# Blaok/soda

Hardware: AMD Instinct MI355X
Metric: stencil cells*iters/s, jacobi2d 8192x8192 iterate=100 (higher is better)
Workload: dtype f32; 1 GPU; jacobi2d float 8192x8192 iterate=100; kernel_family=march2d, decomposition=none, overlap=False, transport=none

## Files before the change

soda_amd/codegen/hip/lower.py:

```python
import dataclasses
import os
from typing import Dict, Optional, Sequence, Union

from soda_amd import core, util

from soda_amd.codegen.hip.module import (KernelDesc, Module, PassDesc,
                                         _check_native, runtime_text)
from soda_amd.codegen.hip.direct import DIRECT_BLOCK, add_direct_pass
from soda_amd.codegen.hip.ldswin import (add_ldswin_pass,
                                         ldswin_candidate, ldswin_pays,
                                         ldswin_supported)
from soda_amd.codegen.hip.march import (LANE_SHIFTS, MAX_FUSE_3D,
                                        MAX_FUSE_PRESERVE, MAX_SHIFT_TEMPS,
                                        MAX_UNROLL, REG_BUDGET, MarchConfig,
                                        add_march_pass, default_vec,
                                        march_supported)
from soda_amd.codegen.hip.tile3d import (add_tile3d_pass,
                                         tile3d_supported)


MAX_TENSORS = 16
DEFAULT_FUSE = (13, 12, 8, 4)
SLIDING_SUMS = os.environ.get('SODA_HIP_SLIDE', '1') != '0'

# ... 5 lines not shown
class LowerOptions:

  strategy: str = 'auto'
  fuse: Sequence[int] = (4,)
  vec: Optional[int] = None
  chunk_rows: Optional[int] = None
  prefetch: Optional[int] = None
  waves_x: int = 1
  waves_y: int = 1
  nt_store: Optional[bool] = None
  nt_load: Optional[bool] = None
  xcd_swizzle: bool = True
  edge_loads: bool = True
  tile_rows: Optional[int] = None
  lane_shift: Optional[str] = None
  min_waves: int = 0
  occupancy: int = 0
  pipe: Optional[int] = None
  pipe_rows: int = 2
  reg_budget: Optional[int] = None
  stamps: bool = False
  peel: Union[None, int, Dict[int, int]] = None
  align_lanes: Optional[int] = None
  xshare: Optional[bool] = None
  row_cells: Optional[int] = None
  xshare_block: Optional[int] = None
  windows: Optional[bool] = None
  inline: Optional[bool] = None
  tile3d_w: Optional[int] = None
  tile3d_h: Optional[int] = None
  tile3d_waves: Optional[int] = None
  banks: Optional[Dict[str, int]] = None
  bank_lead: Optional[Dict[str, int]] = None
  batch: bool = False

  def __post_init__(self):
    self.fuse = tuple(self.fuse)
    if self.inline is None:
      self.inline = os.environ.get('SODA_HIP_INLINE', '1') != '0'
    if self.windows is None:
      self.windows = os.environ.get('SODA_HIP_WINDOWS', '1') != '0'
    if self.xshare is None and os.environ.get('SODA_HIP_XSHARE'):
      self.xshare = os.environ['SODA_HIP_XSHARE'] == '1'
    if self.xshare_block is None and os.environ.get('SODA_HIP_XSHARE_BLOCK'):
      self.xshare_block = int(os.environ['SODA_HIP_XSHARE_BLOCK'])
    if self.align_lanes is None and os.environ.get('SODA_HIP_ALIGN_LANES'):
      self.align_lanes = int(os.environ['SODA_HIP_ALIGN_LANES'])

  def resolved(self, dim: int, iterated: bool = True) -> 'LowerOptions':
    out = dataclasses.replace(self)
    if out.prefetch is None and dim == 3:
      out.prefetch = 1
    if out.nt_load is None:
      out.nt_load = dim != 3 and iterated
    if out.nt_store is None:
      out.nt_store = not iterated
    if out.tile_rows is None:
      out.tile_rows = 4
    return out


NARROW_STRIP_OPS = (48, 128)


def prefers_narrow_strips(stencil: core.Stencil) -> bool:
  if os.environ.get('SODA_HIP_NARROW', '1') == '0':
    return False
  if stencil.dim != 2 or stencil.iterate != 1:
    return False
  if any(str(t) != 'float' for t in stencil.symbol_table.values()):
    return False
  from soda_amd import ir as _ir
  work = sum(_ir.op_count(s.stmt.expr) +
             sum(_ir.op_count(l.expr) for l in s.stmt.let)
             for s in stencil.ordered_stages)
  return NARROW_STRIP_OPS[0] <= work < NARROW_STRIP_OPS[1]


# ... 83 lines not shown
      skip = ((0, None),) + (((stencil.dim - 1, '+'),) if SLIDING_SUMS else ())
    derived = windows.decompose(stencil, skip=skip)
    if len(derived.symbol_table) + len(derived.param_stmts) <= MAX_TENSORS \
        and same_boxes(derived):
      stencil = derived
  from soda_amd.codegen.hip import exact
  stencil = exact.specialize(stencil)
  mod = Module(stencil, opts.banks, opts.batch)
  use_march = opts.strategy in ('auto', 'march', 'tile3d') and \
      march_supported(stencil) is None
  if opts.strategy == 'march' and not use_march:
    raise util.SemanticError('march: %s' % march_supported(stencil))
  if use_march:
    vec0 = opts.vec or default_vec(stencil)
    iterable = (len(stencil.input_names) == len(stencil.output_names) and
                stencil.input_types == stencil.output_types)
    cap = stencil.iterate
    if stencil.dim == 3 and opts.strategy != 'march':
      cap = min(cap, MAX_FUSE_3D)
    if stencil.preserve_border and opts.strategy != 'march':
      cap = min(cap, MAX_FUSE_PRESERVE)
    depths = sorted({min(t, cap) for t in opts.fuse if iterable} - {0, 1},
                    reverse=True)
    if opts.strategy == 'tile3d':
      depths = []

    def peel_for(t: int) -> int:
      if opts.peel is None:
        return -1
      if isinstance(opts.peel, dict):
        return int(opts.peel.get(t, -1))
      return int(opts.peel)

    def pipe_for(t: int) -> int:
      want = default_pipe(t) if opts.pipe is None else opts.pipe
      ok = (want > 1 and t > 1 and t % want == 0 and
            opts.waves_x * opts.waves_y == 1)
      return want if ok else 1

    out_bytes = min(t.size_in_bytes for t in stencil.output_types)

    def shift_for(t: int, xshare: int = 0) -> str:
      if opts.lane_shift is not None:
        return opts.lane_shift
      if xshare or pipe_for(t) > 1 or opts.waves_x * opts.waves_y != 1:
        return 'dpp'
      return default_lane_shift(t, stencil.dim)

    def config(t: int, vec: int, pf: Optional[int],
               rows: Optional[int] = None, xshare: int = 0,
               xshare_block: int = 0) -> MarchConfig:
      shift = shift_for(t, xshare or xshare_block)
      if pf is None:
        pf = default_prefetch(t, shift)
      if opts.align_lanes is not None:
        align = opts.align_lanes
      else:
        align = max(1, 64 // (vec * out_bytes)) if opts.nt_store else 1
      cfg = MarchConfig(
          fused_iters=t, vec=vec, chunk_rows=opts.chunk_rows or 64,
          prefetch=pf, waves_x=opts.waves_x, waves_y=opts.waves_y,
          nt_store=opts.nt_store, nt_load=opts.nt_load,
          xcd_swizzle=opts.xcd_swizzle, edge_loads=opts.edge_loads,
          tile_rows=rows or opts.tile_rows, lane_shift=shift,
          min_waves=opts.min_waves, occupancy=opts.occupancy,
          pipe=pipe_for(t), pipe_rows=opts.pipe_rows, stamps=opts.stamps,
          peel=peel_for(t), align_lanes=align, xshare=xshare,
          xshare_block=xshare_block,
          xwindow=bool(opts.windows),
          slide=bool(opts.windows) and SLIDING_SUMS,
          banks=opts.banks, bank_lead=opts.bank_lead)
      cfg.chunk_fixed = opts.chunk_rows is not None
      return cfg

    budget = opts.reg_budget or REG_BUDGET
    first = default_prefetch(1) if stencil.dim == 2 and work < 128 else \
        (2 if stencil.dim == 2 else 1)
    pfs = [opts.prefetch] if opts.prefetch else [first, 2, 1]
    pfs = sorted(set(pfs), reverse=True)
    rows_list = [opts.tile_rows]
    vecs = []
    v = vec0
    while v >= 1:
      vecs.append(v)
      v //= 2
    chosen = None
    last_error = None
    for v in vecs:
      for rows in rows_list:
        for pf in pfs:
          trial = Module(stencil, opts.banks, opts.batch)
          try:
            est = add_march_pass(trial, config(1, v, pf, rows)).traffic_model[
                'est_window_regs']
          except util.SemanticError as e:
            last_error = e
            continue
          if chosen is None or est < chosen[0]:
            chosen = (est, v, pf, rows)
          if est <= budget:
            break
# ... 73 lines not shown
```

soda_amd/codegen/hip/march.py:

```python
from typing import Dict, List, Optional, Tuple

from soda_amd import core, ir, util

from soda_amd.codegen.hip.module import KernelDesc, Module, PassDesc

MAX_UNROLL = 24
MAX_FUSE_PRESERVE = 8
MAX_FUSE_3D = 2
MAX_SHIFT_TEMPS = 64
REG_BUDGET = 160


class _Node:

  def __init__(self, key, ctype: str, stage: Optional[core.Stage], it: int):
    self.key = key
    self.ctype = ctype
    self.stage = stage
    self.it = it
    self.parents: Dict[str, '_Node'] = {}
    self.delay = 0
    self.first_use = None
    self.window = 1
    self.slots = 1
# ... 25 lines not shown
  @property
  def fill_delay(self) -> int:
    if self.mirror_of is not None:
      return self.delay - MIRROR_PREFETCH
    return 0 if self.stage is None else self.delay

  @property
  def var(self) -> str:
    if self.mirror_of is not None:
      return 'm%d_%s' % (self.owner, self.mirror_of.var)
    if self.stage is None:
      return 'g_%s' % self.key[1]
    return 't%d_%s' % (self.it, self.stage.name)


LDS_PER_CU = 160 * 1024
MIRROR_PREFETCH = 1


LANE_SHIFTS = {'dpp': '', 'mixh': '_mixh'}


class MarchConfig:

  def __init__(self, *, fused_iters: int = 1, vec: int = 4, chunk_rows: int = 64,
               prefetch: int = 2, waves_x: int = 1, waves_y: int = 1,
               nt_store: bool = False, nt_load: bool = True,
               xcd_swizzle: bool = True, edge_loads: bool = True,
               tile_rows: int = 6, lane_shift: str = 'dpp',
               min_waves: int = 0, occupancy: int = 0,
               pipe: int = 1, pipe_rows: int = 4, stamps: bool = False,
               peel: int = -1, align_lanes: int = 1, xshare: int = 0,
               xwindow: bool = True, slide: bool = True,
               xshare_block: int = 0,
               banks: Optional[Dict[str, int]] = None,
               bank_lead: Optional[Dict[str, int]] = None):
    self.banks = dict(banks or {})
    self.bank_lead = {n: int(v) for n, v in (bank_lead or {}).items() if v}
    self.xwindow = xwindow
    self.slide = slide
    self.xshare = int(xshare)
    self.xshare_block = int(xshare_block)
    self.align_lanes = max(1, int(align_lanes))
    self.peel = int(peel)
    self.stamps = stamps
    self.pipe_rows = pipe_rows if pipe > 1 else 1
    self.pipe = pipe
    self.occupancy = occupancy
    self.min_waves = min_waves
    self.lane_shift = lane_shift
    self.fused_iters = fused_iters
    self.vec = vec
    self.chunk_rows = chunk_rows
    self.prefetch = prefetch
    self.waves_x = waves_x
    self.waves_y = waves_y
    self.nt_store = nt_store
    self.nt_load = nt_load
    self.xcd_swizzle = xcd_swizzle
    self.edge_loads = edge_loads
    self.tile_rows = tile_rows
    self.chunk_fixed = False

  def key(self) -> str:
    return ''.join((
        'T%d_V%d_P%d_W%dx%d_R%d' % (self.fused_iters, self.vec, self.prefetch,
                                    self.waves_x, self.waves_y, self.tile_rows),
        '_nts' if self.nt_store else '', '_ntl' if self.nt_load else '',
        '_xcd' if self.xcd_swizzle else '', '_edge' if self.edge_loads else '',
        LANE_SHIFTS[self.lane_shift],
        '_mw%d' % self.min_waves if self.min_waves else '',
        '_occ%d' % self.occupancy if self.occupancy else '',
        '_buf',
        '_pipe%dx%d' % (self.pipe, self.pipe_rows) if self.pipe > 1 else '',
        '_st' if self.stamps else '',
        '_k%d' % self.peel if self.peel >= 0 else '',
        '_al%d' % self.align_lanes if self.align_lanes > 1 else '',
        '_xs%d' % self.xshare if self.xshare and not self.xshare_block
        else '',
        '_xb%d' % self.xshare_block if self.xshare_block else '',
        '_bk_' + '_'.join('%sx%d' % (n, nb) + (
            'l%d' % self.bank_lead[n] if n in self.bank_lead else '')
                         for n, nb in sorted(self.banks.items()))
        if self.banks else ''))


def default_vec(stencil: core.Stencil) -> int:
  widest = max(t.size_in_bytes for t in stencil.symbol_table.values())
  return max(1, 16 // widest)


def bank_fragment_map(vec: int, nb: int) -> List[Tuple[int, int]]:
  if nb < 1 or vec % nb:
    raise util.SemanticError(
        'banks: %d cells per lane are no whole number of groups of %d banks' %
        (vec, nb))
  return [(j % nb, j // nb) for j in range(vec)]


def edge_cell_banks(i: int, vec: int, nb: int) -> Tuple[int, int]:
  if nb < 1 or vec % nb:
    raise util.SemanticError('banks: %d cells per lane, %d banks' % (vec, nb))
  return (-1 - i) % nb, (vec + i) % nb


def march_supported(stencil: core.Stencil) -> Optional[str]:
  if stencil.dim not in (2, 3):
    return 'the marching kernels need a 2- or 3-dimensional program'
  return None


def _build_chain(st: core.Stencil, T: int, pf: int, edge: Tuple[int, int],
                 pipe: int = 1, pipe_rows: int = 1, xshare: bool = False):
# ... 128 lines not shown

  def __init__(self, mod: Module, cfg: MarchConfig):
    self.mod, self.cfg = mod, cfg
    self.st = self.mod.stencil
    why = march_supported(self.st)
    if why:
      raise util.SemanticError('march: %s' % why)
    self.dim = self.st.dim
    self.ax = self.dim - 1
    self.T, self.V, self.PF = self.cfg.fused_iters, self.cfg.vec, self.cfg.prefetch
    if self.T > 1 and len(self.st.input_names) != len(self.st.output_names):
      raise util.SemanticError('march: cannot fuse iterations of a program '
                               'whose inputs and outputs differ in number')
    self.edge = (0, 0)
    self.group = 32 if self.cfg.lane_shift == 'mixh' else 64
    if self.cfg.edge_loads and self.cfg.lane_shift == 'dpp':
      lo = hi = 0
      for stage in self.st.ordered_stages:
        for pname in stage.taps:
          if pname in self.st.input_names:
            tlo, thi = stage.tap_bounds(pname)
            lo, hi = max(lo, -tlo[0]), max(hi, thi[0])
      if max(lo, hi) <= min(self.V, 2):
        self.edge = (lo, hi)
    self.W = self.cfg.pipe
    if self.W > 1:
      if self.T % self.W or self.cfg.waves_x * self.cfg.waves_y != 1:
        raise util.SemanticError(
            'march: %d pipelined waves need a fusion depth that is a multiple '
            'of it and one strip per block' % self.W)
      self.edge = (0, 0)
    self.R = self.cfg.pipe_rows if self.W > 1 else 1
    self.banks = self.cfg.banks
    for nme, nb in self.banks.items():
      if self.mod.banks.get(nme) != nb:
        raise util.InternalError('march: banks of `%s` and the module\'s slots '
                                 'differ' % nme)
      if self.W > 1:
        raise util.SemanticError(
            'march: stage-pipelined blocks read and write dense arrays')
      bank_fragment_map(self.V, nb)
    for nme in self.cfg.bank_lead:
      if nme not in self.banks or nme not in self.st.input_names or \
          self.cfg.bank_lead[nme] % self.banks[nme] or \
          self.cfg.bank_lead[nme] < 0:
        raise util.SemanticError(
            'march: bank_lead of `%s`: a banked input, a multiple of its bank '
            'count' % nme)
    if self.R & (self.R - 1):
      raise util.SemanticError('march: rows per barrier must be a power of two')
    self.xs = self.cfg.xshare
    self.seg = bool(self.cfg.xshare_block)
    if self.seg:
      if not 2 <= self.cfg.xshare_block <= 16:
        raise util.SemanticError(
            'march: xshare_block = %d: 2 to 16 waves share a segment of a row'
            % self.cfg.xshare_block)
      self.xs = self.cfg.xshare_block
    if self.xs:
      self.edge = (0, 0)
      if self.W > 1 or self.cfg.lane_shift != 'dpp' or \
          self.cfg.waves_x * self.cfg.waves_y != 1:
        raise util.SemanticError(
            'march: x-halo sharing needs DPP shifts and one wave per strip')
      if not 1 <= self.xs <= 16:
        raise util.SemanticError('march: 1 to 16 waves can share a row')
# ... 173 lines not shown
    self.w('}')
    return self._finish()

  def _emit_header(self) -> None:
    self.w('// %s: T=%d fused iteration(s), %d cells/lane, chunks of %d along dim %d,'
      ' prefetch %d, unroll %d' % (self.kind, self.T, self.V,
                                   self.cfg.chunk_rows, self.ax, self.PF,
                                   self.U))
    self.w('// strip: %d lanes valid of 64 (halo %d+%d cells, edge loads %d+%d); '
      'pipeline depth %d' % (self.strip_lanes, self.margin_lo, self.margin_hi,
                             self.edge[0], self.edge[1],
                             self.warm))
    if self.seg:
      self.w('// segment: %d waves side by side store %d cells; x-halos shared '
             'through LDS between them, %d+%d halo lanes at the outer sides' %
             (self.xs, self.seg_cells, self.lanes_lo, self.lanes_hi))
    for nme, nb in sorted(self.banks.items()):
      self.w('// banked: %s on %d banks (a.buf[%d..%d]), cell j of a fragment = '
             'element j / %d of bank j %% %d%s' %
             (nme, nb, self.mod.slot[nme], self.mod.slot[nme] + nb - 1, nb, nb,
              ', read %d elements on' % self.cfg.bank_lead[nme]
              if nme in self.cfg.bank_lead else ''))
    if self.dim == 3:
      self.w('// tile: %d rows held in registers for %d output rows (halo %d+%d)' %
        (self.rows_in, self.tile_rows, self.rhalo_lo, self.rhalo_hi))
    for n in self.nodes:
      self.w('//   %-24s delay %2d  window %2d (slots %2d)  margin %d/%d  rows %d/%d' %
        (n.var, n.delay, n.window, n.slots, n.margin[0], n.margin[1],
         n.rmargin[0], n.rmargin[1]))
    self.w('extern "C" __global__ void __launch_bounds__(%d) %s%s(soda_hip_kargs_t a) {'
      % (self.block, '__attribute__((amdgpu_waves_per_eu(%d, %d))) ' %
         (self.cfg.min_waves, max(self.cfg.min_waves, 8))
         if self.cfg.min_waves else '', self.name))
    if self.cfg.stamps:
      self.w('  const unsigned long long soda_t0 = __builtin_amdgcn_s_memtime();')
    self.w('  const int lane = (int)(threadIdx.x & 63u);')
    self.w('  const int wave = __builtin_amdgcn_readfirstlane((int)(threadIdx.x >> 6));')
    if self.cfg.xcd_swizzle:
      self.w('  const unsigned nblk = gridDim.x;')
      self.w('  const unsigned bid = (nblk % 8u == 0u) ? (blockIdx.x % 8u) * (nblk / 8u)'
        ' + blockIdx.x / 8u : blockIdx.x;')
    else:
      self.w('  const unsigned bid = blockIdx.x;')
    self.w('  const int tile_x = (int)(bid % (unsigned)a.ntile[0]);')
    if self.dim == 2:
      self.w('  const int tile_l = (int)(bid / (unsigned)a.ntile[0]);')
      self.w('  const int tile_m = tile_l + (tile_l >= a.skip_from ? a.skip_count : 0);')
      if self.xs:
        self.w('  const int strip = wave;')
        self.w('  const int chunk = tile_m;')
      elif self.W > 1:
        self.w('  const int strip = tile_x;')
        self.w('  const int chunk = tile_m;')
      else:
        self.w('  const int strip = tile_x * %d + wave %% %d;' % (self.wx, self.wx))
        self.w('  const int chunk = tile_m * %d + wave / %d;' % (self.cfg.waves_y, self.wx))
      self.w('  const int n0 = a.extent[0], nm = a.extent[1];')
    else:
      self.w('  const int tile_y = (int)((bid / (unsigned)a.ntile[0]) % '
        '(unsigned)a.ntile[1]);')
      self.w('  const int chunk_l = (int)(bid / ((unsigned)a.ntile[0] * '
        '(unsigned)a.ntile[1]));')
      self.w('  const int chunk = chunk_l + (chunk_l >= a.skip_from ? a.skip_count : 0);')
      self.w('  const int strip = %s;' % ('wave' if self.xs else 'tile_x'))
      self.w('  const int n0 = a.extent[0], n1 = a.extent[1], nm = a.extent[2];')
      self.w('  const int y0 = tile_y * %d - %d;  // first row held' %
# ... 8 lines not shown
      self.w('  const int x0 = strip * %d + (lane - %d) * %d;' %
        (self.strip_cells, self.lanes_lo, self.V))
    else:
      self.w('  const int sub = lane & %d;' % (self.group - 1))
      self.w('  const int x0 = strip * %d + (lane >> 5) * %d + (sub - %d) * %d;'
        % (self.strip_cells, self.group_lanes * self.V, self.lanes_lo, self.V))
    self.w('  const int chunk_len = a.tile[%d] / %d;' %
      (self.ax, self.cfg.waves_y if self.dim == 2 else 1))
    self.w('  const int m_begin = chunk * chunk_len;')
    self.w('  const int m_end = min(m_begin + chunk_len, nm);')
    if self.xs:
      self.w('  if (m_begin >= nm) return;  // block-uniform')
    else:
      self.w('  if (m_begin >= nm || strip * %d >= n0) return;  // wave-uniform' %
        self.strip_cells)
    self.w('  const bool lane_ok = x0 >= 0 && x0 + %d <= n0;' % self.V)
    if self.seg:
      self.w('  const bool store_ok = lane_ok && (strip > 0 || sub >= %d) && '
             '(strip < %d || sub < %d);' %
             (self.lanes_lo, self.xs - 1, 64 - self.lanes_hi))
    else:
      self.w('  const bool store_ok = lane_ok && sub >= %d && sub < %d;' %
        (self.lanes_lo, self.group - self.lanes_hi))
    self.w('  const int64_t pitch = a.stride[%d];' % self.ax)
    self.w('  const int64_t x0c = lane_ok ? (int64_t)x0 : 0;')

  def _emit_addressing(self) -> None:
    table0 = self.st.symbol_table
    self.esz = {nme: table0[nme].size_in_bytes for nme in list(self.inputs) + list(self.outputs)}
    self.n_edge = max(self.edge)
    self.w('  const int in_end = min(nm, m_end + %d);  // last input plane needed + 1'
      % self.m_hi)
    self.w('  const int wlo = max(0, m_begin + (%d));' % self.m_lo)
    for es in sorted(set(self.esz.values())):
      self.w('  const unsigned xb%d = lane_ok ? (unsigned)x0 * %du : SODA_OOB_X;' %
        (es, es))
      self.w('  const unsigned sxb%d = store_ok ? (unsigned)x0 * %du : SODA_OOB_X;' %
        (es, es))
      self.w('  const unsigned pitch_b%d = (unsigned)pitch * %du;' % (es, es))
      if self.dim == 3:
        self.w('  const unsigned pitch_yb%d = (unsigned)pitch_y * %du;' % (es, es))
        for j in range(self.rows_in):
          self.w('  const unsigned yo%d_%d = (y0 + %d >= 0 && y0 + %d < n1) ? '
                 '(unsigned)(y0 + %d) * pitch_yb%d : SODA_OOB_X;' %
                 (es, j, j, j, j, es))
    for nme, n in self.inputs.items():
      if nme in self.banks:
        nb, lead = self.banks[nme], self.cfg.bank_lead.get(nme, 0)
        size = '(int64_t)(in_end - wlo) * pitch'
        if lead:
          self.w('  const int64_t left_%s = (int64_t)a.reserved[0] - %d - '
                 '(int64_t)wlo * pitch;  // elements of the stream from wlo on'
                 % (nme, lead))
          size = '(%s < left_%s ? %s : left_%s)' % (size, nme, size, nme)
        for b in range(nb):
          self.w('  const soda_rsrc_t r_%s_b%d = soda_make_rsrc_bank<%d>((const '
                 '%s*)a.buf[%d] + ((int64_t)wlo * pitch + %d) / %d, %s * %d);' %
                 (nme, b, nb, n.ctype, self.mod.slot[nme] + b, lead, nb, size,
                  self.esz[nme]))
        continue
      self.w('  const soda_rsrc_t r_%s = soda_make_rsrc((const %s*)a.buf[%d] + '
        '(int64_t)wlo * pitch, (int64_t)(in_end - wlo) * pitch * %d);' %
        (nme, n.ctype, self.mod.slot[nme], self.esz[nme]))
    for o, n in self.outputs.items():
      if o in self.banks:
        nb = self.banks[o]
        for b in range(nb):
          self.w('  const soda_rsrc_t w_%s_b%d = soda_make_rsrc_bank<%d>((%s*)'
                 'a.buf[%d] + ((int64_t)m_begin * pitch) / %d, (int64_t)(m_end - '
                 'm_begin) * pitch * %d);' %
                 (o, b, nb, n.ctype, self.mod.slot[o] + b, nb, self.esz[o]))
        continue
      self.w('  const soda_rsrc_t w_%s = soda_make_rsrc((%s*)a.buf[%d] + '
        '(int64_t)m_begin * pitch, (int64_t)(m_end - m_begin) * pitch * %d);' %
        (o, n.ctype, self.mod.slot[o], self.esz[o]))
    if self.xs or self.n_edge:
      self.w('  const bool edge_lane = lane == 0 || lane == 63;')
    self.xs_nodes = [n for n in self.nodes if n.xs]
    if self.xs_nodes:
      self.xs_rows = max(len(self.rows_of(n)) for n in self.xs_nodes)
      if self.xs_rows > 32:
        raise util.SemanticError('march: x-halo sharing holds a row per lane')
      self.xs_stride = self.xs * 2 * self.xs_rows
      for n in self.xs_nodes:
        self.w('  __shared__ %s soda_xs_%s[%d];' %
               (n.ctype, n.var, 2 * self.xs_stride + 1))
      self.w('  if (threadIdx.x == 0) {')
      for n in self.xs_nodes:
        self.w('    soda_xs_%s[%d] = (%s)0;' % (n.var, 2 * self.xs_stride, n.ctype))
      self.w('  }')
      self.w('  soda_pipe_barrier();')
      self.w('  const int xs_wr = (wave * 2 + (lane == 0 ? 0 : 1)) * %d;' %
             self.xs_rows)
      self.w('  const int xs_nb = lane < 32 ? wave - 1 : wave + 1;')
      self.w('  const int xs_rd = (xs_nb >= 0 && xs_nb < %d && (lane & 31) < %d) ? '
             '(xs_nb * 2 + (lane < 32 ? 1 : 0)) * %d + (lane & 31) : %d;' %
             (self.xs, self.xs_rows, self.xs_rows, 2 * self.xs_stride))
    if self.n_edge:
      for i in range(self.n_edge):
        self.w('  const int ex%d = lane == 0 ? x0 - %d : x0 + %d;' %
          (i, 1 + i, self.V + i))
        self.w('  const bool edge_ok%d = edge_lane && ex%d >= 0 && ex%d < n0;' %
          (i, i, i))
        for es in sorted({self.esz[nme] for nme in self.inputs}):
          self.w('  const unsigned exb%d_%d = edge_ok%d ? (unsigned)ex%d * %du : '
            'SODA_OOB_X;' % (i, es, i, i, es))

    if self.st.preserve_border:
      for o in self.st.output_names:
        wlo, whi = self.st.interior_bounds(o)
        for e in range(self.V):
          self.w('  const bool keepx_%s_%d = !(a.origin[0] + x0 + %d >= %d && '
                 'a.origin[0] + x0 + %d < a.gextent[0] - %d);'
                 % (o, e, e, max(0, -wlo[0]), e, max(0, whi[0])))
    self.use_mix = self.cfg.lane_shift == 'mixh'
    self.slide: Dict[int, Tuple[str, Tuple[int, ...], int]] = {}
    if self.cfg.xwindow and self.cfg.slide and self.W == 1:
      from soda_amd.optimization import windows
      table = dict(self.st.symbol_table)
      for n in self.nodes:
        if n.stage is None or n.mirror_of is not None or n.keep is not None:
          continue
        m = windows._match(n.stage.stmt, table)
        if m is None or m[0] != '+' or m[2] != self.ax:
          continue
        off = tuple(a - b for a, b in zip(m[5], n.stage.st_idx))
        self.slide[id(n)] = (m[1], off, m[4])
    declared = set()
    for stage in self.st.ordered_stages:
      for line in self.mod.param_decls(stage):
        if line not in declared:
          declared.add(line)
          self.w(line)
    for n in self.nodes:
      if n.to_lds:
        self.w('  __shared__ %s soda_ring_%s[%d][%d][%d];' % (
            n.ctype, n.var, 2 * self.R, self.rows_in, 64 * self.V))
    self.nt_l = 'true' if self.cfg.nt_load else 'false'
    self.nt_s = 'true' if self.cfg.nt_store else 'false'

  def emit_decls(self, wv: int) -> None:
      for n in self.nodes:
        if n.owner != wv:
          continue
        if id(n) in self.slide:
          for j in self.rows_of(n):
            self.w('  int xa_%s_r%d[%d];' % (n.var, j, self.V))
            self.w('  soda_zero_frag<int, %d>(xa_%s_r%d);' % (self.V, n.var, j))
        for s in range(n.slots):
          for j in self.rows_of(n):
            self.w('  %s %s_s%d_r%d[%d];' % (n.ctype, n.var, s, j, self.V))
            self.w('  soda_zero_frag<%s, %d>(%s_s%d_r%d);' % (n.ctype, self.V, n.var, s, j))
            if n.is_input and self.n_edge:
              self.w('  %s %s_s%d_r%d_e[%d];' % (n.ctype, n.var, s, j, self.n_edge))
              self.w('  soda_zero_frag<%s, %d>(%s_s%d_r%d_e);' %
                (n.ctype, self.n_edge, n.var, s, j))
          if n.xs:
            self.w('  %s hv_%s_s%d = (%s)0;' % (n.ctype, n.var, s, n.ctype))

  def emit_loads(self, k: int, t_expr: str, pin: bool = False) -> None:
      self.w('      const int t = %s;' % t_expr)
      self.w('      const bool plane_ok = t >= 0 && t < in_end;')
      if pin:
        for es in sorted({self.esz[nme] for nme in self.inputs}):
          self.w('      unsigned xb%dp = xb%d; asm volatile("" : "+v"(xb%dp));'
                 % (es, es, es))
      pinned = 'p' if pin else ''
      for es in sorted({self.esz[nme] for nme in self.inputs}):
        if self.dim == 2:
          self.w('      const unsigned ro%d = plane_ok ? (unsigned)(t - wlo) * '
            'pitch_b%d : SODA_OOB_ROW;' % (es, es))
        else:
          self.w('      const unsigned po%d = plane_ok ? (unsigned)(t - wlo) * '
            'pitch_b%d : SODA_OOB_X;' % (es, es))
          for j in sorted({j for n in self.inputs.values() for j in self.rows_of(n)}):
            self.w('      const unsigned ro%d_%d = po%d + yo%d_%d;' %
                   (es, j, es, es, j))
      for nme, n in self.inputs.items():
        s = self.slot_of(n, k, 0)
        for j in self.rows_of(n):
          es = self.esz[nme]
          ro = 'ro%d' % es if self.dim == 2 else 'ro%d_%d' % (es, j)
          reg = '%s_s%d_r%d' % (n.var, s, j)
          if nme in self.banks:
            nb = self.banks[nme]
            self.w('      soda_buf_load_frag_banked<%s, %d, %d, %s>(%s, %s + '
                   'xb%d%s, %s);' %
                   (n.ctype, self.V, nb, self.nt_l, reg, ro, es, pinned,
                    ', '.join('r_%s_b%d' % (nme, b) for b in range(nb))))
            for i in range(self.n_edge):
              left, right = edge_cell_banks(i, self.V, nb)
              self.w('      { %s e1[1], e2[1]; soda_buf_load_cell_banked<%s, %d>('
                     'e1, r_%s_b%d, lane == 0 ? %s + exb%d_%d : SODA_OOB_X); '
                     'soda_buf_load_cell_banked<%s, %d>(e2, r_%s_b%d, lane == 0 '
                     '? SODA_OOB_X : %s + exb%d_%d); %s_e[%d] = lane == 0 ? '
                     'e1[0] : e2[0]; }' %
                     (n.ctype, n.ctype, nb, nme, left, ro, i, es,
                      n.ctype, nb, nme, right, ro, i, es, reg, i))
            continue
          self.w('      soda_buf_load_frag<%s, %d, %s>(%s, r_%s, %s + xb%d%s);' %
            (n.ctype, self.V, self.nt_l, reg, nme, ro, es, pinned))
          for i in range(self.n_edge):
# ... 58 lines not shown
    self._wide: Dict[str, str] = {}
    self._stage_mark = len(self.L)
    fresh_xs: List[Tuple[_Node, int]] = []
    if self.xs and wv == 0:
      for n in self.inputs.values():
        if n.xs:
          fresh_xs.append((n, self.slot_of(n, k, self.PF)))
      for n in self.nodes:
        if not n.xs:
          continue
        slot = self.slot_of(n, k - 1, self.PF if n.is_input else 0)
        self.w('      hv_%s_s%d = soda_xs_%s[xs_rd < %d ? xs_rd + ((t - 1) & 1) * %d '
               ': xs_rd];' % (n.var, slot, n.var, 2 * self.xs_stride,
                              self.xs_stride))
    for n in self.nodes:
      if n.stage is not None and n.owner == wv:
        if step is not None and not self.stage_needed(n, step):
          continue
        first = step is not None and (step == 0 or
                                      not self.stage_needed(n, step - 1))
        self._emit_stage(n, k, slide_init='first' if first else None)
        if n.xs:
          fresh_xs.append((n, self.slot_of(n, k, 0)))
    self.shift_temps = max(self.shift_temps, len(self._shifted))
    if fresh_xs:
      self.w('      if (edge_lane) {')
      for n, slot in fresh_xs:
        for jj, j in enumerate(self.rows_of(n)):
          reg = '%s_s%d_r%d' % (n.var, slot, j)
          self.w('        soda_xs_%s[xs_wr + (t & 1) * %d + %d] = lane == 0 ? %s[0] '
                 ': %s[%d];' % (n.var, self.xs_stride, jj, reg, reg, self.V - 1))
      self.w('      }')
      self.w('      soda_pipe_barrier();')
    self.w('    }')

  def _emit_stage(self, n: _Node, k: int,
                  slide_init: Optional[str] = None) -> None:
    stage = n.stage
    pre: List[str] = []
    early: List[str] = []

    def operand(pname: str, off: Tuple[int, ...], j: int, e: int, _n=n,
                _k=k, _pre=pre, _early=early) -> str:
      p = _n.parents[pname]
      age = _n.delay - off[self.ax] - p.fill_delay
      slot = self.slot_of(p, _k, age)
      row = j + (off[1] if self.dim == 3 else 0)
      if row < p.rmargin[0] or row >= self.rows_in - p.rmargin[1]:
        raise util.InternalError('march: row %d of %s is not held' %
                                 (row, p.var))
      reg = '%s_s%d_r%d' % (p.var, slot, row)
      c = e + off[0]
      lane_off, sub = c // self.V, c % self.V
      src = '%s[%d]' % (reg, sub)
      byte = p.ctype in ('uint8_t', 'int8_t')

      def wide(text: str, tag: str) -> str:
        if not byte:
          return text
        if tag not in self._wide:
          self._wide[tag] = 'w%d_%s' % (len(self._wide), tag)
          _pre.append('      const int %s = soda_wide(%s);' %
                      (self._wide[tag], text))
        return self._wide[tag]

      if lane_off == 0:
# ... 171 lines not shown
            mid = '%s((%s)%s, %s)' % (fn, pt, c, mid)
          body.append('        const %s xm_%s = %s;' % (pt, btag, mid))
          suf = {}
          prev = None
          for i in range(lo - 1, e0 - 1, -1):
            name = 'xs_%s_%d' % (btag, i)
            expr = '(%s)%s' % (pt, cells[i]) if prev is None else \
                '%s((%s)%s, %s)' % (fn, pt, cells[i], prev)
            body.append('        const %s %s = %s;' % (pt, name, expr))
            suf[i] = prev = name
          pre = {}
          prev = None
          for i in range(hi + 1, e0 + b + taps - 1):
            name = 'xp_%s_%d' % (btag, i)
            expr = '(%s)%s' % (pt, cells[i]) if prev is None else \
                '%s(%s, (%s)%s)' % (fn, prev, pt, cells[i])
            body.append('        const %s %s = %s;' % (pt, name, expr))
            pre[i] = prev = name
          for e in range(e0, e0 + b):
            parts = ['xm_%s' % btag]
            if e < lo:
              parts.append(suf[e])
            if e + taps - 1 > hi:
              parts.append(pre[e + taps - 1])
            expr = parts[0]
            for q in parts[1:]:
              expr = '%s(%s, %s)' % (fn, expr, q)
            body.append('        %s = (%s)(%s);' % (dst[e], n.ctype, expr))
      body.append('      }')

  def _emit_store(self, n: _Node, oname: str, dst_slot: int) -> None:
    es = self.esz[oname]
    self.w('      {')
    self.w('        const int m = t - %d;' % n.delay)
    self.w('        const bool m_ok = m >= m_begin && m < m_end;')
    for j in self.store_rows(n):
      reg = '%s_s%d_r%d' % (n.var, dst_slot, j)
      if oname in self.banks:
        nb = self.banks[oname]
        off = ('(m_ok ? (unsigned)(m - m_begin) * pitch_b%d : SODA_OOB_X) + '
               'yo%d_%d + sxb%d' % (es, es, j, es)) if self.dim == 3 else (
                   '(m_ok ? (unsigned)(m - m_begin) * pitch_b%d : SODA_OOB_ROW) '
                   '+ sxb%d' % (es, es))
        self.w('        soda_buf_store_frag_banked<%s, %d, %d, %s>(%s, %s, %s);' %
               (n.ctype, self.V, nb, self.nt_s, off, reg,
                ', '.join('w_%s_b%d' % (oname, b) for b in range(nb))))
        continue
      if self.dim == 3:
        self.w('        soda_buf_store_frag<%s, %d, %s>(w_%s, (m_ok ? (unsigned)'
          '(m - m_begin) * pitch_b%d : SODA_OOB_X) + yo%d_%d + sxb%d, %s);' %
          (n.ctype, self.V, self.nt_s, oname, es, es, j, es, reg))
      else:
        self.w('        soda_buf_store_frag<%s, %d, %s>(w_%s, (m_ok ? '
          '(unsigned)(m - m_begin) * pitch_b%d : SODA_OOB_ROW) + sxb%d, '
          '%s);' % (n.ctype, self.V, self.nt_s, oname, es, es, reg))
    self.w('      }')

  def _finish(self) -> PassDesc:
    if self.shift_temps > MAX_SHIFT_TEMPS:
      raise util.SemanticError(
          'march: %d lane-shifted operands per row step (> %d); the taps reach '
          'too far along dim 0 for %d cells per lane' %
          (self.shift_temps, MAX_SHIFT_TEMPS, self.V))
    self.est_regs += self.shift_temps
    stages = [n for n in self.nodes if n.stage is not None]
    per_wave = []
# ... 7 lines not shown
        wide = 2.0 if n.ctype in ('double', 'int64_t', 'uint64_t') else 1.0
        ops += cost * wide * self.V * len(self.rows_of(n))
      per_wave.append(ops + 8.0)
    step_ops = max(per_wave)
    saved = sum(1 for i in range(self.peeled) for n in stages
                if not self.stage_needed(n, i)) / float(max(1, len(stages)))
    if self.dim == 2:
      tile = (self.strip_cells * (self.xs or self.wx),
              self.cfg.chunk_rows * self.cfg.waves_y)
    else:
      tile = (self.strip_cells * (self.xs or 1), self.tile_rows,
              self.cfg.chunk_rows)
    if self.seg:
      tile = (self.seg_cells,) + tile[1:]
    lds_pad = 0
    if self.cfg.occupancy:
      blocks_per_cu = max(1, 4 * self.cfg.occupancy // self.waves)
      lds_pad = min(65536, (LDS_PER_CU // (blocks_per_cu + 1)) // 1024 * 1024
                    + 1024)
    idx = self.mod.add_kernel(
        KernelDesc(self.name, (self.block, 1, 1), tile, lds_bytes=lds_pad,
                   note='%s %s' % (self.kind, self.cfg.key()),
                   tune=dict(axis=self.ax, waves_along=self.cfg.waves_y if self.dim == 2 else 1,
                             waves_per_block=self.waves, warm=self.warm,
                             fixed=self.cfg.chunk_fixed, occupancy=self.cfg.occupancy,
                             pipe=self.W, vec=self.V, step_ops=step_ops,
                             lane_shift=self.cfg.lane_shift,
                             warm_saved=saved,
                             lane_redundancy=self.lane_redundancy,
                             peel_trips=self.peeled // self.U,
                             unroll=self.U, tile_rows=self.tile_rows,
                             peel_trips_max=self.peel_trips_max,
                             fused=self.T,
                             window_extra=self.m_hi - self.m_lo,
                             max_elem=max(self.esz.values()),
                             max_extent0=0 if self.seg else
                             self.strip_cells * self.xs)),
        '\n'.join(self.L) + '\n')
    table = self.st.symbol_table
    bytes_in = sum(table[i].size_in_bytes for i in self.st.input_names)
    bytes_out = sum(table[o].size_in_bytes for o in self.st.output_names)
    redundancy = self.lane_redundancy * (
        (self.cfg.chunk_rows + self.warm) / float(self.cfg.chunk_rows)) * (
            self.rows_in / float(self.tile_rows))
    p = PassDesc(
        self.T, [idx], self.kind,
        dict(bytes_per_cell_min=bytes_in + bytes_out,
             read_redundancy=redundancy, strip_cells=self.strip_cells, warm_rows=self.warm,
             unroll=self.U, edge=self.edge, rows_in=self.rows_in, tile_rows=self.tile_rows,
             est_window_regs=self.est_regs))
    self.mod.passes.append(p)
    return p


def add_march_pass(mod: Module, cfg: MarchConfig) -> PassDesc:
  return _MarchKernel(mod, cfg).emit()
```

soda_amd/csrc/soda_rt.h:

```cpp

#ifdef __HIPCC_RTC__
typedef __INT8_TYPE__ int8_t;
typedef __UINT8_TYPE__ uint8_t;
typedef __INT16_TYPE__ int16_t;
typedef __UINT16_TYPE__ uint16_t;
typedef __INT32_TYPE__ int32_t;
typedef __UINT32_TYPE__ uint32_t;
typedef __INT64_TYPE__ int64_t;
typedef __UINT64_TYPE__ uint64_t;
#else
#include <hip/hip_runtime.h>
#include <stdint.h>
#endif

struct soda_hip_kargs_t {
  void* buf[16];
  int64_t stride[4];
  int32_t extent[4];
  int32_t ntile[4];
  int32_t tile[4];
  int32_t origin[4];
  int32_t gextent[4];
  int32_t skip_from;
  int32_t skip_count;
// ... 228 lines not shown
    for (int e = 0; e < V; ++e) dst[e] = t[e];
  }
}

template <class T, int V>
SODA_DEV void soda_zero_frag(T (&dst)[V]) {
#pragma unroll
  for (int e = 0; e < V; ++e) dst[e] = (T)0;
}

template <class T, int V, bool kNonTemporal = false>
SODA_DEV void soda_store_frag(T* __restrict__ p, const T (&src)[V]) {
  if constexpr (V == 1) {
    if constexpr (kNonTemporal) __builtin_nontemporal_store(src[0], p);
    else *p = src[0];
  } else {
    typedef typename soda_vec<T, V>::type vec_t;
    vec_t t;
#pragma unroll
    for (int e = 0; e < V; ++e) t[e] = src[e];
    if constexpr (kNonTemporal)
      __builtin_nontemporal_store(t, reinterpret_cast<vec_t*>(p));
    else
      *reinterpret_cast<vec_t*>(p) = t;
  }
}

typedef unsigned soda_u32x4 __attribute__((ext_vector_type(4)));
typedef unsigned soda_u32x2 __attribute__((ext_vector_type(2)));
typedef __amdgpu_buffer_rsrc_t soda_rsrc_t;
#define SODA_OOB_X 0x40000000u
#define SODA_OOB_ROW 0x80000000u
#define SODA_BUF_WINDOW_MAX 0x40000000ll

SODA_DEV soda_rsrc_t soda_make_rsrc(const void* base, int64_t bytes) {
  return __builtin_amdgcn_make_buffer_rsrc(
      const_cast<void*>(base), 0,
      (int)(bytes < 0 ? 0 : bytes > SODA_BUF_WINDOW_MAX ? SODA_BUF_WINDOW_MAX
                                                        : bytes),
      0x00020000);
}

template <class T, int V, bool kNonTemporal = false>
SODA_DEV void soda_buf_load_frag(T (&dst)[V], soda_rsrc_t r, unsigned off) {
  constexpr int kBytes = V * (int)sizeof(T);
  constexpr int kAux = kNonTemporal ? 2 : 0;
  if constexpr (kBytes % 16 == 0) {
#pragma unroll
    for (int i = 0; i < kBytes / 16; ++i) {
      const soda_u32x4 t =
          __builtin_amdgcn_raw_buffer_load_b128(r, off + 16 * i, 0, kAux);
      __builtin_memcpy((char*)dst + 16 * i, &t, 16);
    }
  } else if constexpr (kBytes == 8) {
    const soda_u32x2 t = __builtin_amdgcn_raw_buffer_load_b64(r, off, 0, kAux);
    __builtin_memcpy(dst, &t, 8);
  } else if constexpr (kBytes == 4) {
    const unsigned t = __builtin_amdgcn_raw_buffer_load_b32(r, off, 0, kAux);
    __builtin_memcpy(dst, &t, 4);
  } else if constexpr (kBytes == 2) {
    const unsigned short t =
        __builtin_amdgcn_raw_buffer_load_b16(r, off, 0, kAux);
    __builtin_memcpy(dst, &t, 2);
  } else {
    static_assert(kBytes == 1, "fragment size");
    const unsigned char t = __builtin_amdgcn_raw_buffer_load_b8(r, off, 0, kAux);
// ... 52 lines not shown
```

soda_amd/runtime.py:

```python
import ctypes
import hashlib
import os
from typing import Dict, Optional, Sequence

from soda_amd import core, util
from soda_amd.codegen.hip import lower

_HERE = os.path.dirname(os.path.abspath(__file__))
LIB_PATH = os.environ.get('SODA_HIP_LIBRARY') or \
    os.path.join(_HERE, 'libsoda_hip.so')
CACHE_DIR = os.environ.get('SODA_HIP_CACHE',
                           os.path.join(_HERE, '_jit_cache'))
ARCH = 'gfx950'
COMPILE_OPTIONS = ('--offload-arch=%s' % ARCH, '-O3', '-ffp-contract=off',
                   '-fno-slp-vectorize', '-fwrapv', '-std=c++17') + tuple(
                       os.environ.get('SODA_HIP_EXTRA_FLAGS', '').split())

MAX_DIM = 4
MAX_TENSORS = 16
MAX_KERNELS = 32
MAX_PASSES = 8
MAX_PASS_KERNELS = 16
MAX_PARAMS = 8
MAX_SLABS = 64
# ... 556 lines not shown
  count = (ctypes.c_int32 * plan.num_passes)()
  check(lib.soda_hip_plan_schedule(ctypes.byref(plan), ext, iterate, count),
        'schedule of %d iterations' % iterate)
  return list(count)


def plan_launches(plan: Plan, extent: Sequence[int], iterate: int,
                  run: Optional[SlabRun] = None):
  lib = library()
  ext = (ctypes.c_int32 * MAX_DIM)(*(list(extent) + [1] * (MAX_DIM - len(extent))))
  n = ctypes.c_int32(0)
  cap = 4096
  arr = (LaunchInfo * cap)()
  check(lib.soda_hip_plan_launches(ctypes.byref(plan), ext, iterate,
                                   ctypes.byref(run) if run is not None else
                                   None, cap, arr, ctypes.byref(n)),
        'launches of %d iterations' % iterate)
  return [{name: getattr(arr[i], name) for name, _ in LaunchInfo._fields_}
          for i in range(min(n.value, cap))]


def pick_vec(stencil: core.Stencil, extent: Optional[Sequence[int]]) -> int:
  vec = lower.default_vec(stencil)
  if extent is not None:
    while vec > 1 and extent[0] % vec:
      vec //= 2
  return vec


ICACHE_BYTES = 60 * 1024


def select_peel(stencil: core.Stencil, opts: 'lower.LowerOptions',
                extent: Optional[Sequence[int]] = None) -> Dict[int, int]:
  import copy
  import json
  plain = copy.copy(opts)
  plain.peel = 0
  mod0 = lower.lower(stencil, plain)
  todo = {}
  for k in mod0.kernels:
    if k.tune and k.tune.get('peel_trips_max'):
      todo[k.tune['fused']] = k.tune['peel_trips_max']
  if not todo:
    return {}
  long_chunks = {}
  res0 = kernel_resources(compile_source(mod0.source,
                                         '%s.hip' % stencil.app_name))
  if extent is not None:
    try:
      tiles, _ = plan_geometry(make_plan(mod0, res0), extent)
      for k, tile in zip(mod0.kernels, tiles):
        if k.tune and k.tune.get('fused') in todo:
          long_chunks[k.tune['fused']] = \
              tile[k.tune['axis']] >= 8 * max(1, k.tune.get('warm') or 1)
    except util.SodaError:
      pass
  key = hashlib.sha256(('peel3\0' + compiler_version() + '\0' +
                        '\0'.join(COMPILE_OPTIONS) + '\0' +
                        repr(sorted(long_chunks.items())) + '\0' +
                        mod0.source).encode()).hexdigest()[:24]
  memo = os.path.join(CACHE_DIR, 'peel_%s.json' % key)
  try:
    with open(memo) as f:
      return {int(t): int(v) for t, v in json.load(f).items()}
  except (OSError, ValueError):
    pass

  def probe(depth: int, trips: int):
    if trips == 0:
      res, mod = res0, mod0
    else:
      one = copy.copy(opts)
      one.fuse = (depth,) if depth > 1 else ()
      one.peel = trips
      mod = lower.lower(stencil, one)
      res = kernel_resources(compile_source(mod.source,
                                            '%s.hip' % stencil.app_name))
    for k in mod.kernels:
      if k.tune and k.tune.get('fused') == depth:
        r = res.get(k.name)
        return None if not r else (waves_per_simd(r['vgpr']), r['scratch'],
                                   r.get('code', 0))
    return None

  chosen = {}
  for depth, most in todo.items():
    base = probe(depth, 0)
    chosen[depth] = 0
    if base is None:
      continue
    for trips in range(most, 0, -1):
      got = probe(depth, trips)
      if got is None or got[0] < base[0] or got[1] > base[1]:
        continue
      if long_chunks.get(depth) and got[2] > ICACHE_BYTES >= base[2]:
        continue
      chosen[depth] = trips
      break
  try:
    os.makedirs(CACHE_DIR, exist_ok=True)
    tmp = '%s.%d.tmp' % (memo, os.getpid())
    with open(tmp, 'w') as f:
      json.dump(chosen, f)
    os.replace(tmp, memo)
  except OSError:
    pass
  return chosen


def select_shape(stencil: core.Stencil, opts: 'lower.LowerOptions',
                 extent: Optional[Sequence[int]] = None):
  import copy
  import json
  if opts.strategy not in ('auto', 'march') or stencil.iterate > 1:
    return None
  if min(t.size_in_bytes for t in stencil.symbol_table.values()) >= 4:
    return None
  base = copy.copy(opts)
  base.peel = 0
  mod0 = lower.lower(stencil, base)
  one = [k for k in mod0.kernels if k.tune and k.tune.get('fused') == 1 and
         'axis' in k.tune]
  if not one:
    return None
  chosen = int(one[0].tune.get('vec') or 1)
  want = int(opts.vec or lower.default_vec(stencil))
  if chosen >= want:
    return None
  key = hashlib.sha256(('shape2\0' + compiler_version() + '\0' +
                        '\0'.join(COMPILE_OPTIONS) + '\0%d\0' % want +
                        mod0.source).encode()).hexdigest()[:24]
  memo = os.path.join(CACHE_DIR, 'shape_%s.json' % key)
  try:
    with open(memo) as f:
      got = json.load(f)
    return tuple(got) if got else None
  except (OSError, ValueError):
    pass
  found = None
# ... 31 lines not shown
                    opts: Optional['lower.LowerOptions'],
                    extent: Optional[Sequence[int]],
                    probe: bool = True) -> 'lower.LowerOptions':
  import copy
  out = copy.copy(opts) if opts is not None else lower.LowerOptions()
  if out.vec is None:
    out.vec = pick_vec(stencil, extent)
    if out.prefetch is None and out.strategy in ('auto', 'march') and \
        lower.prefers_narrow_strips(stencil):
      out.vec, out.prefetch = min(out.vec, 2), 4
  if out.row_cells is None and extent is not None:
    out.row_cells = int(extent[0])
  probing = probe and not os.environ.get('SODA_HIP_NO_PROBE')
  if probing and out.prefetch is None and out.reg_budget is None and \
      out.strategy in ('auto', 'march') and \
      lower.march_supported(stencil) is None:
    try:
      shape = select_shape(stencil, out, extent)
    except (util.SodaError, OSError):
      shape = None
    if shape:
      out.vec, out.prefetch = shape
      out.reg_budget = 1 << 20
  if out.peel is None and out.strategy in ('auto', 'march', 'tile3d') and \
      lower.march_supported(stencil) is None:
    if not probe or os.environ.get('SODA_HIP_NO_PROBE'):
      out.peel = 0
    else:
      asked = out
      if out.strategy == 'tile3d':
        asked = copy.copy(out)
        asked.strategy, asked.fuse = 'auto', ()
      try:
        out.peel = select_peel(stencil, asked, extent)
      except (util.SodaError, OSError):
        out.peel = 0
  return out


def clipped_box(box, extent: Sequence[int]):
  lo = [min(max(l, 0), e) for l, e in zip(box[0], extent)]
  hi = [min(max(h, l), e) for l, h, e in zip(lo, box[1], extent)]
  return lo, hi


class Program:

  def __init__(self, stencil: core.Stencil,
               opts: Optional[lower.LowerOptions] = None, device: int = 0,
               extent: Optional[Sequence[int]] = None,
               calibrate: Optional[bool] = None,
               source_prefix: str = ''):
    self.stencil = stencil
    self.opts = resolve_options(stencil, opts, extent)
    self.device = device
    self.module = lower.lower(stencil, self.opts)
    self.code = compile_source(source_prefix + self.module.source,
                               '%s.hip' % stencil.app_name)
    self.resources = kernel_resources(self.code)
    self.plan = make_plan(self.module, self.resources)
    if extent is not None:
      self.geometry(extent)
    self._lib = library()
    self._handle = ctypes.c_void_p()
    check(
        self._lib.soda_hip_program_create(self.code, len(self.code),
                                          ctypes.byref(self.plan), device,
# ... 580 lines not shown
```

Before: 5864 billion cells*iters/s.

## Carry row offsets incrementally in march kernels and add VGPR floor padding

In 2D single-wave march kernels without banks, per-iteration plane bounds checks and row-offset multiplies are replaced by running load/store row offsets that are clamped to a cap, so out-of-range rows fall outside the buffer window instead of being tested. Store guards on m are dropped in the same way. A separate VGPR floor knob pins a high register with an empty asm clobber. It is chosen automatically for deep-warm mixh kernels that sit at three waves, padding them to a register count that holds occupancy at two waves, likely to cut cache contention. Both options are enabled by default and change peel-cache keys; they rely on buffer-resource range checks being correct for the clamped offsets.

```diff
diff --git a/soda_amd/codegen/hip/lower.py b/soda_amd/codegen/hip/lower.py
--- a/soda_amd/codegen/hip/lower.py
+++ b/soda_amd/codegen/hip/lower.py
@@ -61,6 +61,8 @@
   tile3d_waves: Optional[int] = None
   banks: Optional[Dict[str, int]] = None
   bank_lead: Optional[Dict[str, int]] = None
+  row_carry: Optional[bool] = None
+  vgpr_floor: Union[None, int, Dict[int, int]] = None
   batch: bool = False
 
   def __post_init__(self):
@@ -73,6 +75,8 @@
       self.xshare = os.environ['SODA_HIP_XSHARE'] == '1'
     if self.xshare_block is None and os.environ.get('SODA_HIP_XSHARE_BLOCK'):
       self.xshare_block = int(os.environ['SODA_HIP_XSHARE_BLOCK'])
+    if self.row_carry is None:
+      self.row_carry = os.environ.get('SODA_HIP_ROW_CARRY', '1') != '0'
     if self.align_lanes is None and os.environ.get('SODA_HIP_ALIGN_LANES'):
       self.align_lanes = int(os.environ['SODA_HIP_ALIGN_LANES'])
 
@@ -222,6 +226,11 @@
         return int(opts.peel.get(t, -1))
       return int(opts.peel)
 
+    def floor_for(t: int) -> int:
+      if isinstance(opts.vgpr_floor, dict):
+        return int(opts.vgpr_floor.get(t, 0))
+      return int(opts.vgpr_floor or 0)
+
     def pipe_for(t: int) -> int:
       want = default_pipe(t) if opts.pipe is None else opts.pipe
       ok = (want > 1 and t > 1 and t % want == 0 and
@@ -256,7 +265,8 @@
           min_waves=opts.min_waves, occupancy=opts.occupancy,
           pipe=pipe_for(t), pipe_rows=opts.pipe_rows, stamps=opts.stamps,
           peel=peel_for(t), align_lanes=align, xshare=xshare,
-          xshare_block=xshare_block,
+          xshare_block=xshare_block, row_carry=bool(opts.row_carry),
+          vgpr_floor=floor_for(t),
           xwindow=bool(opts.windows),
           slide=bool(opts.windows) and SLIDING_SUMS,
           banks=opts.banks, bank_lead=opts.bank_lead)
diff --git a/soda_amd/codegen/hip/march.py b/soda_amd/codegen/hip/march.py
--- a/soda_amd/codegen/hip/march.py
+++ b/soda_amd/codegen/hip/march.py
@@ -81,10 +81,13 @@
                pipe: int = 1, pipe_rows: int = 4, stamps: bool = False,
                peel: int = -1, align_lanes: int = 1, xshare: int = 0,
                xwindow: bool = True, slide: bool = True,
-               xshare_block: int = 0,
+               xshare_block: int = 0, row_carry: bool = True,
+               vgpr_floor: int = 0,
                banks: Optional[Dict[str, int]] = None,
                bank_lead: Optional[Dict[str, int]] = None):
     self.banks = dict(banks or {})
+    self.row_carry = bool(row_carry)
+    self.vgpr_floor = int(vgpr_floor)
     self.bank_lead = {n: int(v) for n, v in (bank_lead or {}).items() if v}
     self.xwindow = xwindow
     self.slide = slide
@@ -128,6 +131,8 @@
         '_xs%d' % self.xshare if self.xshare and not self.xshare_block
         else '',
         '_xb%d' % self.xshare_block if self.xshare_block else '',
+        '' if self.row_carry else '_rc0',
+        '_vf%d' % self.vgpr_floor if self.vgpr_floor else '',
         '_bk_' + '_'.join('%sx%d' % (n, nb) + (
             'l%d' % self.bank_lead[n] if n in self.bank_lead else '')
                          for n, nb in sorted(self.banks.items()))
@@ -322,6 +327,8 @@
       self.edge = (0, 0)
     self.R = self.cfg.pipe_rows if self.W > 1 else 1
     self.banks = self.cfg.banks
+    self.carry = (self.cfg.row_carry and self.dim == 2 and self.W == 1 and
+                  not self.banks)
     for nme, nb in self.banks.items():
       if self.mod.banks.get(nme) != nb:
         raise util.InternalError('march: banks of `%s` and the module\'s slots '
@@ -561,6 +568,9 @@
       % (self.block, '__attribute__((amdgpu_waves_per_eu(%d, %d))) ' %
          (self.cfg.min_waves, max(self.cfg.min_waves, 8))
          if self.cfg.min_waves else '', self.name))
+    if self.cfg.vgpr_floor > 1:
+      self.w('  asm volatile("" ::: "v%d");  // MarchConfig.vgpr_floor' %
+             (min(self.cfg.vgpr_floor, 256) - 1))
     if self.cfg.stamps:
       self.w('  const unsigned long long soda_t0 = __builtin_amdgcn_s_memtime();')
     self.w('  const int lane = (int)(threadIdx.x & 63u);')
@@ -635,12 +645,18 @@
     self.w('  const int in_end = min(nm, m_end + %d);  // last input plane needed + 1'
       % self.m_hi)
     self.w('  const int wlo = max(0, m_begin + (%d));' % self.m_lo)
+    oob_x = self.oob_x = 'SODA_OOB_ROW' if self.carry else 'SODA_OOB_X'
     for es in sorted(set(self.esz.values())):
-      self.w('  const unsigned xb%d = lane_ok ? (unsigned)x0 * %du : SODA_OOB_X;' %
-        (es, es))
-      self.w('  const unsigned sxb%d = store_ok ? (unsigned)x0 * %du : SODA_OOB_X;' %
-        (es, es))
+      self.w('  const unsigned xb%d = lane_ok ? (unsigned)x0 * %du : %s;' %
+        (es, es, oob_x))
+      self.w('  const unsigned sxb%d = store_ok ? (unsigned)x0 * %du : %s;' %
+        (es, es, oob_x))
       self.w('  const unsigned pitch_b%d = (unsigned)pitch * %du;' % (es, es))
+      if self.carry:
+        self.w('  const int row_cap%d = SODA_ROW_CAP - (int)pitch_b%d;' % (es, es))
+        if es in {self.esz[nme] for nme in self.inputs}:
+          self.w('  int rl%d = (m_begin + (%d) - wlo) * (int)pitch_b%d;' %
+                 (es, self.m_lo, es))
       if self.dim == 3:
         self.w('  const unsigned pitch_yb%d = (unsigned)pitch_y * %du;' % (es, es))
         for j in range(self.rows_in):
@@ -677,6 +693,10 @@
       self.w('  const soda_rsrc_t w_%s = soda_make_rsrc((%s*)a.buf[%d] + '
         '(int64_t)m_begin * pitch, (int64_t)(m_end - m_begin) * pitch * %d);' %
         (o, n.ctype, self.mod.slot[o], self.esz[o]))
+    if self.carry:
+      for o, n in self.outputs.items():
+        self.w('  int rs_%s = (%d) * (int)pitch_b%d;' %
+               (o, self.m_lo + self.lead - n.delay, self.esz[o]))
     if self.xs or self.n_edge:
       self.w('  const bool edge_lane = lane == 0 || lane == 63;')
     self.xs_nodes = [n for n in self.nodes if n.xs]
@@ -707,7 +727,7 @@
           (i, i, i))
         for es in sorted({self.esz[nme] for nme in self.inputs}):
           self.w('  const unsigned exb%d_%d = edge_ok%d ? (unsigned)ex%d * %du : '
-            'SODA_OOB_X;' % (i, es, i, i, es))
+            '%s;' % (i, es, i, i, es, oob_x))
 
     if self.st.preserve_border:
       for o in self.st.output_names:
@@ -763,14 +783,19 @@
 
   def emit_loads(self, k: int, t_expr: str, pin: bool = False) -> None:
       self.w('      const int t = %s;' % t_expr)
-      self.w('      const bool plane_ok = t >= 0 && t < in_end;')
+      if not self.carry:
+        self.w('      const bool plane_ok = t >= 0 && t < in_end;')
       if pin:
         for es in sorted({self.esz[nme] for nme in self.inputs}):
           self.w('      unsigned xb%dp = xb%d; asm volatile("" : "+v"(xb%dp));'
                  % (es, es, es))
       pinned = 'p' if pin else ''
       for es in sorted({self.esz[nme] for nme in self.inputs}):
-        if self.dim == 2:
+        if self.carry:
+          self.w('      const unsigned ro%d = (unsigned)rl%d;' % (es, es))
+          self.w('      rl%d = min(rl%d, row_cap%d) + (int)pitch_b%d;' %
+                 (es, es, es, es))
+        elif self.dim == 2:
           self.w('      const unsigned ro%d = plane_ok ? (unsigned)(t - wlo) * '
             'pitch_b%d : SODA_OOB_ROW;' % (es, es))
         else:
@@ -895,6 +920,11 @@
                  ': %s[%d];' % (n.var, self.xs_stride, jj, reg, reg, self.V - 1))
       self.w('      }')
       self.w('      soda_pipe_barrier();')
+    if self.carry:
+      for o, n in self.outputs.items():
+        if n.owner == wv:
+          self.w('      rs_%s = min(rs_%s, row_cap%d) + (int)pitch_b%d;' %
+                 (o, o, self.esz[o], self.esz[o]))
     self.w('    }')
 
   def _emit_stage(self, n: _Node, k: int,
@@ -1132,6 +1162,13 @@
   def _emit_store(self, n: _Node, oname: str, dst_slot: int) -> None:
     es = self.esz[oname]
     self.w('      {')
+    if self.carry:
+      for j in self.store_rows(n):
+        self.w('        soda_buf_store_frag<%s, %d, %s>(w_%s, (unsigned)rs_%s + '
+               'sxb%d, %s_s%d_r%d);' % (n.ctype, self.V, self.nt_s, oname,
+                                        oname, es, n.var, dst_slot, j))
+      self.w('      }')
+      return
     self.w('        const int m = t - %d;' % n.delay)
     self.w('        const bool m_ok = m >= m_begin && m < m_end;')
     for j in self.store_rows(n):
@@ -1205,7 +1242,8 @@
                              unroll=self.U, tile_rows=self.tile_rows,
                              peel_trips_max=self.peel_trips_max,
                              fused=self.T,
-                             window_extra=self.m_hi - self.m_lo,
+                             window_extra=max(self.m_hi - self.m_lo, self.warm)
+                             if self.carry else self.m_hi - self.m_lo,
                              max_elem=max(self.esz.values()),
                              max_extent0=0 if self.seg else
                              self.strip_cells * self.xs)),
diff --git a/soda_amd/csrc/soda_rt.h b/soda_amd/csrc/soda_rt.h
--- a/soda_amd/csrc/soda_rt.h
+++ b/soda_amd/csrc/soda_rt.h
@@ -284,6 +284,7 @@
 #define SODA_OOB_X 0x40000000u
 #define SODA_OOB_ROW 0x80000000u
 #define SODA_BUF_WINDOW_MAX 0x40000000ll
+#define SODA_ROW_CAP 0x40000000
 
 SODA_DEV soda_rsrc_t soda_make_rsrc(const void* base, int64_t bytes) {
   return __builtin_amdgcn_make_buffer_rsrc(
diff --git a/soda_amd/runtime.py b/soda_amd/runtime.py
--- a/soda_amd/runtime.py
+++ b/soda_amd/runtime.py
@@ -612,16 +612,21 @@
 
 
 def select_peel(stencil: core.Stencil, opts: 'lower.LowerOptions',
-                extent: Optional[Sequence[int]] = None) -> Dict[int, int]:
+                extent: Optional[Sequence[int]] = None,
+                floors: Optional[Dict[int, int]] = None) -> Dict[int, int]:
   import copy
   import json
   plain = copy.copy(opts)
   plain.peel = 0
   mod0 = lower.lower(stencil, plain)
   todo = {}
+  warm = {}
   for k in mod0.kernels:
     if k.tune and k.tune.get('peel_trips_max'):
       todo[k.tune['fused']] = k.tune['peel_trips_max']
+      if k.tune.get('lane_shift') == 'mixh' and \
+          k.tune.get('waves_per_block', 1) == 1:
+        warm[k.tune['fused']] = k.tune.get('warm') or 0
   if not todo:
     return {}
   long_chunks = {}
@@ -636,15 +641,18 @@
               tile[k.tune['axis']] >= 8 * max(1, k.tune.get('warm') or 1)
     except util.SodaError:
       pass
-  key = hashlib.sha256(('peel3\0' + compiler_version() + '\0' +
+  key = hashlib.sha256(('peel7\0' + compiler_version() + '\0' +
                         '\0'.join(COMPILE_OPTIONS) + '\0' +
                         repr(sorted(long_chunks.items())) + '\0' +
                         mod0.source).encode()).hexdigest()[:24]
   memo = os.path.join(CACHE_DIR, 'peel_%s.json' % key)
   try:
     with open(memo) as f:
-      return {int(t): int(v) for t, v in json.load(f).items()}
-  except (OSError, ValueError):
+      saved = json.load(f)
+    if floors is not None:
+      floors.update({int(t): int(v) for t, v in saved['floor'].items()})
+    return {int(t): int(v) for t, v in saved['peel'].items()}
+  except (OSError, ValueError, KeyError, TypeError):
     pass
 
   def probe(depth: int, trips: int):
@@ -665,6 +673,7 @@
     return None
 
   chosen = {}
+  floor = {}
   for depth, most in todo.items():
     base = probe(depth, 0)
     chosen[depth] = 0
@@ -677,15 +686,20 @@
       if long_chunks.get(depth) and got[2] > ICACHE_BYTES >= base[2]:
         continue
       chosen[depth] = trips
+      base = got
       break
+    if warm.get(depth, 0) > 12 and base[0] == 3:
+      floor[depth] = 512 // (8 * 3) * 8 + 1
   try:
     os.makedirs(CACHE_DIR, exist_ok=True)
     tmp = '%s.%d.tmp' % (memo, os.getpid())
     with open(tmp, 'w') as f:
-      json.dump(chosen, f)
+      json.dump({'peel': chosen, 'floor': floor}, f)
     os.replace(tmp, memo)
   except OSError:
     pass
+  if floors is not None:
+    floors.update(floor)
   return chosen
 
 
@@ -783,7 +797,10 @@
         asked = copy.copy(out)
         asked.strategy, asked.fuse = 'auto', ()
       try:
-        out.peel = select_peel(stencil, asked, extent)
+        floors = {}
+        out.peel = select_peel(stencil, asked, extent, floors)
+        if out.vgpr_floor is None and floors:
+          out.vgpr_floor = floors
       except (util.SodaError, OSError):
         out.peel = 0
   return out
```

Result: no change. 5920 billion cells*iters/s, median of 6 (+0.9%).
